# allenai/OLMoASR

Hardware: AMD Instinct MI355X
Metric: audio-seconds/sec/node (train step) (higher is better)
Workload: dtype bf16

## Files before the change

include/oasr_testing.h:

```cpp
#ifndef OASR_TESTING_H
#define OASR_TESTING_H
#include "oasr.h"
#ifdef __cplusplus
extern "C" {
#endif

int oasr_profile_gemm(int enable);
int oasr_gemm_set_variant(int v);
int oasr_decode_set_ln_fold(int mode);
int oasr_span_set_side_streams(int mode);
int oasr_span_side_streams(void);
int oasr_xcd_plan_debug(int d, int H, int Te, int M, int L, int team, int wg, int* out, int max_blocks);
int oasr_wide_supports_debug(int d, int H, int Te, int S_max, int L, int M, int nwg);
int oasr_wide_plan_debug(int d, int nwg, int N, int K, int wg, int wave, int* out, int max_units);
int oasr_xcd_offsets_ok_debug(const int64_t* layer0, long long lstride, long long cache_lstride, int d, int Te, int L, int M);
int oasr_attention_set_pingpong(int on);
int oasr_attention_set_span_grid(int on);
int oasr_gemm_set_stagger(int sleeps, int phases);
int oasr_gemm_force_general(int on);
int oasr_test_gemm(const oasr_gemm_args* a, float* colsum_scratch, int atomic_on_pp, int raster_gm, int stagger, int stagger_phases, void* stream);
int oasr_profile_gemm_records(char* buf, int cap);
int oasr_profile_gemm_collect(double* ms4, double* flops4, int64_t* count4, char* by_symbol , int cap);
int oasr_probe_lds_oob(const void* src_u16 , void* dst_u16 , void* stream);
int oasr_probe_tr16(const void* src_bf16 , void* dst_bf16 , void* stream);
int oasr_test_span_tables(const int32_t* span_host, int B, int S, const int64_t* targets, int32_t* rows_out, int32_t* span_out,
                          int64_t* targets_rows_out, int64_t* active_rows_out, void* stream);
int oasr_test_span_block_tables(const int32_t* span_host, int B, int S, int H, const int64_t* targets, int32_t* rows_out, int32_t* span_out,
                                int64_t* targets_rows_out, int32_t* blk128_out, int32_t* blk256_out, int32_t* counts_out, void* stream);

int oasr_test_embedding_fwd(const int64_t* tok, const float* E, const float* pos, void* x, int dtype, int B, int S, int d, int64_t n_embed,
                            const int32_t* rows, void* stream);
int oasr_test_embedding_bwd(const int64_t* tok, const void* dx, int dtype, float* dE, float* dpos, int B, int S, int d, int64_t pad_id,
                            int64_t n_embed, const int32_t* rows, const int32_t* span, void* stream);
int oasr_test_colsum(const void* x, int dtype, int64_t ld, int64_t M, int ncols, float* out, void* stream);
int oasr_test_conv2_col2im_dgelu(const void* dA, const void* u1, void* dpre1, int dtype, int B, int T1, int d, void* stream);
int oasr_test_conv1_col2im_mel(const void* dcol, int dtype, float* dmel, int B, int T1, int n_mels, void* stream);
int oasr_test_mel_to_time_major(const float* mel, void* out, int dtype, int B, int n_mels, int T, const float* clip_max, void* stream);
int oasr_test_pack_conv_weight(const float* w, void* dst, int dtype, int co, int ci, int ldk, void* stream);
int oasr_test_unpack_conv_grad(const float* g, float* dw, int co, int ci, int ldk, void* stream);
int oasr_test_pack_embedding(const float* e, void* dst, int rows, int rows_pad, int d, void* stream);
int oasr_test_dgelu_mul(const void* dy, const void* u, void* out, int dtype, int64_t n, void* stream);
int oasr_test_dlogits_from_f32(const float* src, int V, int64_t rows, int64_t ld, void* dst, int dtype, void* stream);
int oasr_test_logits_to_f32(const void* logits, int dtype, int64_t ld, int64_t rows, int V, float* out, void* stream);
int oasr_test_layernorm_bwd(const void* dy, const void* x, const float* gamma, const float* mean, const float* rstd, const void* dres, void* dx,
                            float* dgamma, float* dbeta, float* dsum, int dtype, int64_t rows, int d, void* stream);

int oasr_test_dtw_host(const float* cost, int64_t ld, int N, int M, int negate, int32_t* text_indices, int32_t* time_indices, int32_t* path_len,
                       void* workspace);

int oasr_test_argmax_rows(const void* logits, int dtype, int64_t ld, int V, int64_t n_rows, const int32_t* rows, const int32_t* span, int B, int S,
                          int32_t* pred_out, void* stream);

#ifdef __cplusplus
}
#endif
#endif
```

olmoasr_amd/_native.py:

```python
import ctypes as C
import os

import torch

_HERE = os.path.dirname(os.path.abspath(__file__))
LIB_PATH = os.environ.get("OASR_LIB") or os.path.join(_HERE, "liboasr.so")
_lib = None


class NativeError(RuntimeError):
    pass


class Dims(C.Structure):
    _fields_ = [(n, C.c_int) for n in ("n_mels", "n_audio_ctx", "n_audio_state", "n_audio_head", "n_audio_layer",
                                       "n_vocab", "n_text_ctx", "n_text_state", "n_text_head", "n_text_layer")]


class Operand(C.Structure):
    _fields_ = [("ptr", C.c_void_p), ("ld", C.c_int64), ("rpb", C.c_int), ("bstride", C.c_int64), ("lead", C.c_int),
                ("kvalid", C.c_int), ("trail_from", C.c_int)]


class GemmArgs(C.Structure):
# ... 25 lines not shown

class SpecAug(C.Structure):
    MAX_MASKS = 8
    _fields_ = [("freq_masks", C.c_int32), ("freq_width", C.c_int32), ("time_masks", C.c_int32), ("time_width", C.c_int32), ("fill", C.c_float)]


class EditArgs(C.Structure):
    MAX_LEN = 1023
    _fields_ = [("hyp", C.c_void_p), ("ref", C.c_void_p), ("hyp_len", C.c_void_p), ("ref_len", C.c_void_p), ("out", C.c_void_p),
                ("ld_hyp", C.c_int64), ("ld_ref", C.c_int64), ("B", C.c_int32), ("Lh", C.c_int32), ("Lr", C.c_int32), ("reserved", C.c_int32)]


class TrainStepArgs(C.Structure):
    _fields_ = [(n, C.c_void_p) for n in ("mel", "xa", "tokens", "targets", "text_len", "span_host", "mel_clip_max", "loss_out", "logits_out",
                                          "pred_out", "seg_events")] + \
               [(n, C.c_int32) for n in ("B", "S", "span_forward", "accumulate_loss")] + [("loss_scale", C.c_float), ("inv_accum", C.c_float)] + \
               [("label_smoothing", C.c_float), ("z_loss", C.c_float), ("loss_parts_out", C.c_void_p), ("loss_parts_rows", C.c_void_p)]


DTW_MAX_N, DTW_MAX_M = 448, 1500
ABI_VERSION = 216
KV_TAIL_BYTES = 327680
MODE_INFER, MODE_TRAIN, MODE_TRAIN_ENC, MODE_TRAIN_DEC = 0, 1, 2, 3
ROWTAB = 16
LORA_MAX_RANK = 64


def _declare(lib):
    vp, i32, i64, f32, sz = C.c_void_p, C.c_int, C.c_int64, C.c_float, C.c_size_t
    sig = {
        "oasr_last_error": (C.c_char_p, []),
        "oasr_version": (i32, []),
        "oasr_log_mel_workspace_bytes": (sz, [i32]),
        "oasr_log_mel": (i32, [vp, i32, i32, i32, vp, vp, vp]),
        "oasr_mel_filterbank": (i32, [vp]),
        "oasr_create": (vp, [C.POINTER(Dims)]),
        "oasr_create_ex": (vp, [C.POINTER(Dims), i32]),
        "oasr_create_ex2": (vp, [C.POINTER(Dims), i32, i32]),
        "oasr_compute_dtype": (i32, [vp]),
        "oasr_create_ex3": (vp, [C.POINTER(Dims), i32, i32, vp, i32, i32, f32]),
        "oasr_lora_count": (i32, [vp]),
        "oasr_lora_merge": (i32, [vp, vp]),
        "oasr_lora_merge_op": (i32, [vp, vp, vp, i32, i32, i32, f32, i32, vp, vp]),
        "oasr_lora_grad_scratch_bytes": (sz, [i32, i32, i32]),
        "oasr_lora_grad_op": (i32, [vp, vp, vp, i32, i32, i32, f32, vp, vp, vp, vp]),
        "oasr_encode": (i32, [vp, vp, i32, vp, vp, sz, vp]),
        "oasr_kv_cache_bytes": (sz, [vp, i32]),
        "oasr_decode_step_workspace_bytes": (sz, [vp, i32]),
        "oasr_decode_begin": (i32, [vp, vp, i32, vp, vp]),
        "oasr_decode_step": (i32, [vp, vp, i32, i32, vp, vp, vp, sz, vp]),
        "oasr_decode_check": (i32, [vp, i32, vp, vp]),
        "oasr_decode_logits": (i32, [vp, vp, vp, vp, i32, i32, i32, vp, vp, sz, vp]),
        "oasr_destroy": (None, [vp]),
        "oasr_param_count": (i32, [vp]),
        "oasr_param_info": (i32, [vp, i32, C.c_char_p, i32, C.POINTER(i64), C.POINTER(i64), C.POINTER(i32), C.POINTER(i64)]),
        "oasr_param_numel": (i64, [vp]),
        "oasr_segment_count": (i32, [vp]),
        "oasr_segment_info": (i32, [vp, i32, C.POINTER(i64), C.POINTER(i64)]),
        "oasr_bind": (i32, [vp, vp, vp, vp, vp, vp]),
        "oasr_shadow_bytes": (sz, [vp]),
        "oasr_bind_shadow": (i32, [vp, vp]),
        "oasr_refresh_shadow": (i32, [vp, vp]),
        "oasr_workspace_bytes": (sz, [vp, i32, i32, i32]),
        "oasr_forward": (i32, [vp, vp, vp, vp, i32, i32, vp, vp, vp, sz, vp]),
        "oasr_sizeof_train_step_args": (sz, []),
        "oasr_train_step": (i32, [vp, C.POINTER(TrainStepArgs), vp, sz, vp]),
        "oasr_log_mel_raw": (i32, [vp, i32, i32, i32, vp, vp, vp, vp]),
        "oasr_sizeof_attn_args": (sz, []),
        "oasr_test_span_tables": (i32, [vp, i32, i32, vp, vp, vp, vp, vp, vp]),
        "oasr_test_span_block_tables": (i32, [vp, i32, i32, i32, vp, vp, vp, vp, vp, vp, vp, vp]),
        "oasr_test_embedding_fwd": (i32, [vp, vp, vp, vp, i32, i32, i32, i32, i64, vp, vp]),
        "oasr_test_embedding_bwd": (i32, [vp, vp, i32, vp, vp, i32, i32, i32, i64, i64, vp, vp, vp]),
        "oasr_test_colsum": (i32, [vp, i32, i64, i64, i32, vp, vp]),
        "oasr_test_conv2_col2im_dgelu": (i32, [vp, vp, vp, i32, i32, i32, i32, vp]),
        "oasr_test_conv1_col2im_mel": (i32, [vp, i32, vp, i32, i32, i32, vp]),
        "oasr_test_mel_to_time_major": (i32, [vp, vp, i32, i32, i32, i32, vp, vp]),
        "oasr_test_pack_conv_weight": (i32, [vp, vp, i32, i32, i32, i32, vp]),
        "oasr_test_unpack_conv_grad": (i32, [vp, vp, i32, i32, i32, vp]),
        "oasr_test_pack_embedding": (i32, [vp, vp, i32, i32, i32, vp]),
        "oasr_test_dgelu_mul": (i32, [vp, vp, vp, i32, i64, vp]),
        "oasr_test_dlogits_from_f32": (i32, [vp, i32, i64, i64, vp, i32, vp]),
        "oasr_test_logits_to_f32": (i32, [vp, i32, i64, i64, i32, vp, vp]),
        "oasr_test_layernorm_bwd": (i32, [vp, vp, vp, vp, vp, vp, vp, vp, vp, vp, i32, i64, i32, vp]),
        "oasr_train_fwd": (i32, [vp, vp, vp, vp, i32, i32, vp, vp, sz, vp]),
        "oasr_train_bwd": (i32, [vp, vp, vp, vp, i32, i32, vp, vp, sz, vp]),
        "oasr_zero_grad": (i32, [vp, vp]),
        "oasr_train_encode": (i32, [vp, vp, i32, vp, vp, sz, vp]),
        "oasr_train_encode_bwd": (i32, [vp, vp, i32, vp, vp, sz, vp]),
        "oasr_train_decode": (i32, [vp, vp, vp, vp, i32, i32, vp, vp, sz, vp]),
        "oasr_train_decode_bwd": (i32, [vp, vp, vp, vp, i32, i32, vp, vp, sz, vp]),
        "oasr_set_trainable": (i32, [vp, vp, i32]),
        "oasr_optim_step": (i32, [vp, f32, f32, f32, f32, f32, f32, f32, i64, vp, vp, vp]),
        "oasr_grad_sumsq_range": (i32, [vp, i64, i64, vp, vp, vp]),
        "oasr_optim_step_range": (i32, [vp, i64, i64, vp, vp, vp, f32, f32, f32, f32, f32, f32, f32, i64, vp]),
        "oasr_gemm": (i32, [C.POINTER(GemmArgs), vp]),
        "oasr_test_gemm": (i32, [C.POINTER(GemmArgs), vp, i32, i32, i32, i32, vp]),
        "oasr_profile_gemm_records": (i32, [C.c_char_p, i32]),
        "oasr_layernorm_fwd": (i32, [vp, vp, vp, vp, vp, vp, i64, i32, vp]),
        "oasr_layernorm_bwd": (i32, [vp, vp, vp, vp, vp, vp, vp, vp, vp, i64, i32, vp]),
        "oasr_attention_fwd": (i32, [C.POINTER(AttnArgs), vp]),
        "oasr_attention_bwd": (i32, [C.POINTER(AttnArgs), vp]),
        "oasr_attention_scores": (i32, [C.POINTER(AttnArgs), i32, vp, vp]),
        "oasr_sizeof_align_args": (sz, []),
        "oasr_alignment_workspace_bytes": (sz, [i32, i32, i32]),
        "oasr_alignment_matrix": (i32, [C.POINTER(AlignArgs), vp, sz, vp]),
        "oasr_dtw_workspace_bytes": (sz, [i32, i32]),
        "oasr_dtw": (i32, [vp, i64, i32, i32, i32, vp, vp, vp, vp, sz, vp]),
        "oasr_test_dtw_host": (i32, [vp, i64, i32, i32, i32, vp, vp, vp, vp]),
        "oasr_sizeof_specaug": (sz, []),
        "oasr_spec_augment": (i32, [vp, i32, i32, i32, C.POINTER(SpecAug), C.c_uint64, C.c_uint64, vp]),
        "oasr_spec_augment_plan": (i32, [C.POINTER(SpecAug), C.c_uint64, C.c_uint64, i32, i32, vp, vp]),
        "oasr_sizeof_edit_args": (sz, []),
        "oasr_edit_counts": (i32, [C.POINTER(EditArgs), vp]),
        "oasr_edit_counts_host": (i32, [C.POINTER(EditArgs)]),
        "oasr_test_argmax_rows": (i32, [vp, i32, i64, i32, i64, vp, vp, i32, i32, vp, vp]),
        "oasr_cross_entropy": (i32, [vp, i64, i32, vp, i64, i64, f32, vp, vp, vp, i32, vp]),
        "oasr_cross_entropy_ex": (i32, [vp, i64, i32, vp, i64, i64, f32, vp, vp, vp, i32, f32, f32, vp, vp]),
        "oasr_cast_f32_bf16": (i32, [vp, vp, i64, vp]),
        "oasr_pick_tokens": (i32, [vp, i64, i32, i64, vp, vp, vp, vp, vp]),
        "oasr_pick_tokens_ts": (i32, [vp, i64, i32, i64, vp, vp, vp, i64, i32, i32, i32, i32, i32, vp, vp, vp]),
        "oasr_topk_tokens": (i32, [vp, i64, i32, i64, vp, vp, vp, i64, i32, i32, i32, i32, i32, i32, vp, vp, vp]),
        "oasr_sample_tokens": (i32, [vp, i64, i32, i64, vp, vp, vp, i64, i32, i32, i32, i32, i32, f32, vp, vp, vp, vp]),
        "oasr_probe_tr16": (i32, [vp, vp, vp]),
        "oasr_probe_lds_oob": (i32, [vp, vp, vp]),
        "oasr_profile_gemm": (i32, [i32]),
        "oasr_gemm_force_general": (i32, [i32]),
        "oasr_gemm_set_stagger": (i32, [i32, i32]),
        "oasr_gemm_set_variant": (i32, [i32]),
        "oasr_decode_set_ln_fold": (i32, [i32]),
        "oasr_span_set_side_streams": (i32, [i32]),
        "oasr_span_side_streams": (i32, []),
        "oasr_xcd_plan_debug": (i32, [i32, i32, i32, i32, i32, i32, i32, vp, i32]),
        "oasr_xcd_offsets_ok_debug": (i32, [vp, C.c_longlong, C.c_longlong, i32, i32, i32, i32]),
        "oasr_wide_supports_debug": (i32, [i32, i32, i32, i32, i32, i32, i32]),
        "oasr_wide_plan_debug": (i32, [i32, i32, i32, i32, i32, i32, vp, i32]),
        "oasr_attention_set_pingpong": (i32, [i32]),
        "oasr_attention_set_span_grid": (i32, [i32]),
        "oasr_profile_gemm_collect": (i32, [vp, vp, vp, C.c_char_p, i32]),
    }
    for name, (res, args) in sig.items():
        fn = getattr(lib, name)
        fn.restype = res
        fn.argtypes = args
    return list(sig)


EXPORTS = None


def lib():
    global _lib, EXPORTS
    if _lib is None:
        if not os.path.isfile(LIB_PATH):
            raise NativeError(f"{LIB_PATH} not found: run `python -c 'import __graft_entry__ as g; g.build()'` "
                              "(hipcc --offload-arch=gfx950).  There is no CPU/PyTorch fallback for this path.")
        try:
            _lib = C.CDLL(LIB_PATH)
        except OSError as e:
            raise NativeError(f"cannot load {LIB_PATH}: {e}") from e
        handle, _lib = _lib, None
        vfn = getattr(handle, "oasr_version", None)
        ver = int(vfn()) if vfn is not None else None
        sfn = getattr(handle, "oasr_sizeof_attn_args", None)
        size = int(sfn()) if sfn is not None else None
        if ver != ABI_VERSION or size != C.sizeof(AttnArgs):
            raise NativeError(f"{LIB_PATH}: ABI version {ver} / oasr_attn_args of {size} bytes, this binding is written for version "
# ... 48 lines not shown
```

olmoasr_amd/csrc/api.hip:

```cpp
#include <stdarg.h>

#include "../../include/oasr.h"
#include "kernels.h"

static thread_local char g_err[512] = "";

void oasr_set_error(const char* fmt, ...) {
  va_list ap;
  va_start(ap, fmt);
  vsnprintf(g_err, sizeof(g_err), fmt, ap);
  va_end(ap);
}

extern "C" const char* oasr_last_error(void) { return g_err; }
extern "C" int oasr_version(void) { return OASR_ABI_VERSION; }
extern "C" size_t oasr_sizeof_attn_args(void) { return sizeof(oasr_attn_args); }

static OperandView to_view(const oasr_operand& o) {
  return OperandView{(const bf16_t*)o.ptr, (long)o.ld, o.rpb, (long)o.bstride, o.lead, o.kvalid, o.trail_from};
}

static int to_gemm(const oasr_gemm_args* a, GemmArgs& g) {
  OASR_REQUIRE(a, "oasr_gemm: null args");
  g = gemm_defaults();
// ... 200 lines not shown
}

#define OASR_TEST_DTYPE(name) \
  OASR_REQUIRE(dtype == OASR_DTYPE_BF16 || dtype == OASR_DTYPE_F32, name ": dtype %d (0 = bf16, 1 = fp32 activations)", dtype)

extern "C" int oasr_test_embedding_fwd(const int64_t* tok, const float* E, const float* pos, void* x, int dtype, int B, int S, int d,
                                       int64_t n_embed, const int32_t* rows, void* stream) {
  OASR_TEST_DTYPE("oasr_test_embedding_fwd");
  if (dtype == OASR_DTYPE_BF16) return launch_embedding_fwd(tok, E, pos, (bf16_t*)x, B, S, d, (long)n_embed, (hipStream_t)stream, rows);
  return launch_embedding_fwd(tok, E, pos, (float*)x, B, S, d, (long)n_embed, (hipStream_t)stream, rows);
}
extern "C" int oasr_test_embedding_bwd(const int64_t* tok, const void* dx, int dtype, float* dE, float* dpos, int B, int S, int d, int64_t pad_id,
                                       int64_t n_embed, const int32_t* rows, const int32_t* span, void* stream) {
  OASR_TEST_DTYPE("oasr_test_embedding_bwd");
  OASR_REQUIRE(!span || rows, "oasr_test_embedding_bwd: span comes with a chunk-row table");
  if (dtype == OASR_DTYPE_BF16)
    return launch_embedding_bwd(tok, (const bf16_t*)dx, dE, dpos, B, S, d, (long)pad_id, (long)n_embed, (hipStream_t)stream, rows, span);
  return launch_embedding_bwd(tok, (const float*)dx, dE, dpos, B, S, d, (long)pad_id, (long)n_embed, (hipStream_t)stream, rows, span);
}
extern "C" int oasr_test_colsum(const void* x, int dtype, int64_t ld, int64_t M, int ncols, float* out, void* stream) {
  OASR_TEST_DTYPE("oasr_test_colsum");
  if (dtype == OASR_DTYPE_BF16) return launch_colsum_accum((const bf16_t*)x, (long)ld, (long)M, ncols, out, (hipStream_t)stream);
  return launch_colsum_accum((const float*)x, (long)ld, (long)M, ncols, out, (hipStream_t)stream);
}
extern "C" int oasr_test_conv2_col2im_dgelu(const void* dA, const void* u1, void* dpre1, int dtype, int B, int T1, int d, void* stream) {
  OASR_TEST_DTYPE("oasr_test_conv2_col2im_dgelu");
  OASR_REQUIRE(B > 0 && T1 > 0 && d > 0, "oasr_test_conv2_col2im_dgelu: bad shape (B=%d T1=%d d=%d)", B, T1, d);
  if (dtype == OASR_DTYPE_BF16) return launch_conv2_col2im_dgelu((const bf16_t*)dA, (const bf16_t*)u1, (bf16_t*)dpre1, B, T1, d, (hipStream_t)stream);
  return launch_conv2_col2im_dgelu((const float*)dA, (const float*)u1, (float*)dpre1, B, T1, d, (hipStream_t)stream);
}
extern "C" int oasr_test_conv1_col2im_mel(const void* dcol, int dtype, float* dmel, int B, int T1, int n_mels, void* stream) {
  OASR_TEST_DTYPE("oasr_test_conv1_col2im_mel");
  if (dtype == OASR_DTYPE_BF16) return launch_conv1_col2im_mel((const bf16_t*)dcol, dmel, B, T1, n_mels, (hipStream_t)stream);
  return launch_conv1_col2im_mel((const float*)dcol, dmel, B, T1, n_mels, (hipStream_t)stream);
}
extern "C" int oasr_test_mel_to_time_major(const float* mel, void* out, int dtype, int B, int n_mels, int T, const float* clip_max, void* stream) {
  OASR_TEST_DTYPE("oasr_test_mel_to_time_major");
  OASR_REQUIRE(B > 0 && n_mels > 0 && T > 0, "oasr_test_mel_to_time_major: bad shape (B=%d n_mels=%d T=%d)", B, n_mels, T);
  if (dtype == OASR_DTYPE_BF16) return launch_mel_to_time_major(mel, (bf16_t*)out, B, n_mels, T, (hipStream_t)stream, clip_max);
  return launch_mel_to_time_major(mel, (float*)out, B, n_mels, T, (hipStream_t)stream, clip_max);
}
extern "C" int oasr_test_pack_conv_weight(const float* w, void* dst, int dtype, int co, int ci, int ldk, void* stream) {
  OASR_TEST_DTYPE("oasr_test_pack_conv_weight");
  OASR_REQUIRE(co > 0 && ci > 0, "oasr_test_pack_conv_weight: bad shape (co=%d ci=%d)", co, ci);
  if (dtype == OASR_DTYPE_BF16) return launch_pack_conv_weight(w, (bf16_t*)dst, co, ci, ldk, (hipStream_t)stream);
  return launch_pack_conv_weight(w, (float*)dst, co, ci, ldk, (hipStream_t)stream);
}
extern "C" int oasr_test_unpack_conv_grad(const float* g, float* dw, int co, int ci, int ldk, void* stream) {
  OASR_REQUIRE(co > 0 && ci > 0, "oasr_test_unpack_conv_grad: bad shape (co=%d ci=%d)", co, ci);
  return launch_unpack_conv_grad(g, dw, co, ci, ldk, (hipStream_t)stream);
}
extern "C" int oasr_test_pack_embedding(const float* e, void* dst, int rows, int rows_pad, int d, void* stream) {
  OASR_REQUIRE(rows > 0 && d > 0, "oasr_test_pack_embedding: bad shape (rows=%d d=%d)", rows, d);
  return launch_pack_embedding(e, (bf16_t*)dst, rows, rows_pad, d, (hipStream_t)stream);
}
extern "C" int oasr_test_dgelu_mul(const void* dy, const void* u, void* out, int dtype, int64_t n, void* stream) {
  OASR_TEST_DTYPE("oasr_test_dgelu_mul");
  OASR_REQUIRE(n > 0, "oasr_test_dgelu_mul: n = %lld", (long long)n);
  if (dtype == OASR_DTYPE_BF16) return launch_dgelu_mul((const bf16_t*)dy, (const bf16_t*)u, (bf16_t*)out, (long)n, (hipStream_t)stream);
  return launch_dgelu_mul((const float*)dy, (const float*)u, (float*)out, (long)n, (hipStream_t)stream);
}
extern "C" int oasr_test_dlogits_from_f32(const float* src, int V, int64_t rows, int64_t ld, void* dst, int dtype, void* stream) {
  OASR_TEST_DTYPE("oasr_test_dlogits_from_f32");
  OASR_REQUIRE(rows > 0 && V > 0, "oasr_test_dlogits_from_f32: bad shape");
  if (dtype == OASR_DTYPE_BF16) return launch_dlogits_from_f32(src, V, (long)rows, (long)ld, (bf16_t*)dst, (hipStream_t)stream);
  return launch_dlogits_from_f32(src, V, (long)rows, (long)ld, (float*)dst, (hipStream_t)stream);
}
extern "C" int oasr_test_logits_to_f32(const void* logits, int dtype, int64_t ld, int64_t rows, int V, float* out, void* stream) {
  OASR_TEST_DTYPE("oasr_test_logits_to_f32");
  OASR_REQUIRE(logits && out && rows > 0 && V > 0 && V <= ld, "oasr_test_logits_to_f32: bad args");
  if (dtype == OASR_DTYPE_BF16) return launch_logits_to_f32((const bf16_t*)logits, (long)ld, (long)rows, V, out, (hipStream_t)stream);
  return launch_logits_to_f32((const float*)logits, (long)ld, (long)rows, V, out, (hipStream_t)stream);
}
extern "C" int oasr_test_layernorm_bwd(const void* dy, const void* x, const float* gamma, const float* mean, const float* rstd, const void* dres,
                                       void* dx, float* dgamma, float* dbeta, float* dsum, int dtype, int64_t rows, int d, void* stream) {
  OASR_TEST_DTYPE("oasr_test_layernorm_bwd");
  if (dtype == OASR_DTYPE_BF16)
    return launch_layernorm_bwd((const bf16_t*)dy, (const bf16_t*)x, gamma, mean, rstd, (const bf16_t*)dres, (bf16_t*)dx, dgamma, dbeta, dsum,
                                (long)rows, d, (hipStream_t)stream);
  return launch_layernorm_bwd((const float*)dy, (const float*)x, gamma, mean, rstd, (const float*)dres, (float*)dx, dgamma, dbeta, dsum, (long)rows, d,
                              (hipStream_t)stream);
}

extern "C" int oasr_test_argmax_rows(const void* logits, int dtype, int64_t ld, int V, int64_t n_rows, const int32_t* rows, const int32_t* span, int B,
                                     int S, int32_t* pred_out, void* stream) {
  OASR_TEST_DTYPE("oasr_test_argmax_rows");
  if (dtype == OASR_DTYPE_BF16)
    return launch_argmax_rows((const bf16_t*)logits, (long)ld, V, (long)n_rows, rows, span, B, S, pred_out, (hipStream_t)stream);
  return launch_argmax_rows((const float*)logits, (long)ld, V, (long)n_rows, rows, span, B, S, pred_out, (hipStream_t)stream);
}

extern "C" int oasr_cross_entropy_ex(void* logits, int64_t ld, int V, const int64_t* targets, int64_t rows, int64_t ignore, float gscale,
                                     int32_t* n_valid_dev, float* row_loss, float* loss_out, int write_grad, float label_smoothing, float z_loss,
                                     float* row_parts, void* stream) {
  hipStream_t st = (hipStream_t)stream;
  int rc = check_ce_reg("oasr_cross_entropy_ex", label_smoothing, z_loss);
  if (rc) return rc;
  CeReg reg;
  reg.eps = label_smoothing;
  reg.z = z_loss;
  reg.parts = row_parts;
  reg.parts_stride = (long)rows;
  rc = launch_count_valid(targets, rows, ignore, V, n_valid_dev, st);
  if (rc) return rc;
  rc = launch_cross_entropy((bf16_t*)logits, ld, V, targets, rows, ignore, gscale, n_valid_dev, row_loss, write_grad, st, reg);
  if (rc) return rc;
  if (loss_out) rc = launch_loss_reduce(row_loss, rows, n_valid_dev, 1.0f, loss_out, 0, st);
  return rc;
}
extern "C" int oasr_cross_entropy(void* logits, int64_t ld, int V, const int64_t* targets, int64_t rows, int64_t ignore, float gscale,
                                  int32_t* n_valid_dev, float* row_loss, float* loss_out, int write_grad, void* stream) {
  return oasr_cross_entropy_ex(logits, ld, V, targets, rows, ignore, gscale, n_valid_dev, row_loss, loss_out, write_grad, 0.f, 0.f, nullptr, stream);
}

extern "C" int oasr_pick_tokens(const float* logits, int64_t ld, int V, int64_t rows, const float* mask, const float* mask2, int64_t* tok,
                                float* logprob, void* stream) {
  return launch_pick_tokens(logits, ld, V, rows, mask, mask2, tok, logprob, (hipStream_t)stream);
}

extern "C" int oasr_pick_tokens_ts(const float* logits, int64_t ld, int V, int64_t rows, const float* mask, const float* mask2,
                                   const int64_t* history, int64_t history_ld, int n_history, int timestamp_begin, int eot, int no_timestamps,
                                   int max_initial_index, int64_t* tok, float* logprob, void* stream) {
  return launch_pick_tokens_ts(logits, ld, V, rows, mask, mask2, history, history_ld, n_history, timestamp_begin, eot, no_timestamps,
                               max_initial_index, tok, logprob, (hipStream_t)stream);
}

extern "C" int oasr_topk_tokens(const float* logits, int64_t ld, int V, int64_t rows, const float* mask, const float* mask2,
                                const int64_t* history, int64_t history_ld, int n_history, int timestamp_begin, int eot, int no_timestamps,
                                int max_initial_index, int K, int64_t* tok, float* logprob, void* stream) {
  return launch_topk_tokens_ts(logits, ld, V, rows, mask, mask2, history, history_ld, n_history, timestamp_begin, eot, no_timestamps,
                               max_initial_index, K, tok, logprob, (hipStream_t)stream);
}
extern "C" int oasr_sample_tokens(const float* logits, int64_t ld, int V, int64_t rows, const float* mask, const float* mask2,
                                  const int64_t* history, int64_t history_ld, int n_history, int timestamp_begin, int eot, int no_timestamps,
                                  int max_initial_index, float temperature, const float* uniforms, int64_t* tok, float* logprob, void* stream) {
  return launch_sample_tokens_ts(logits, ld, V, rows, mask, mask2, history, history_ld, n_history, timestamp_begin, eot, no_timestamps,
                                 max_initial_index, temperature, uniforms, tok, logprob, (hipStream_t)stream);
}

extern "C" int oasr_cast_f32_bf16(const float* src, void* dst, int64_t n, void* stream) {
  return launch_cast_f32_bf16(src, (bf16_t*)dst, n, (hipStream_t)stream);
}

typedef __attribute__((address_space(3))) s16x4_t* lds_s16x4_ptr_t;
__global__ void probe_tr16_kernel(const bf16_t* __restrict__ src, bf16_t* __restrict__ dst) {
  __shared__ __attribute__((aligned(16))) bf16_t tile[16 * 64];
  const int l = threadIdx.x;
  for (int i = l; i < 16 * 64; i += 64) tile[i] = src[i];
  __syncthreads();
  const int row = (l >> 4) * 4 + ((l & 15) >> 2), col = ((l & 15) & 3) * 4;
  const s16x4_t v = __builtin_amdgcn_ds_read_tr16_b64_v4i16((lds_s16x4_ptr_t)(tile + row * 64 + col));
  for (int j = 0; j < 4; ++j) dst[l * 4 + j] = (bf16_t)v[j];
}
typedef __attribute__((address_space(3))) void* lds_void_ptr_t;
__global__ void probe_lds_oob_kernel(const bf16_t* __restrict__ src, bf16_t* __restrict__ dst) {
  __shared__ __attribute__((aligned(16))) bf16_t tile[64 * 8];
  const int l = threadIdx.x;
  for (int i = l; i < 64 * 8; i += 64) tile[i] = 0xAAAA;
  __syncthreads();
  const __amdgpu_buffer_rsrc_t rs = __builtin_amdgcn_make_buffer_rsrc(const_cast<bf16_t*>(src), 0, 64 * 16, 0x00020000);
  const unsigned off = l < 32 ? l * 16 : 0x80000000u;
  __builtin_amdgcn_raw_ptr_buffer_load_lds(rs, (lds_void_ptr_t)tile, 16, off, 0, 0, 0);
  __syncthreads();
  for (int i = l; i < 64 * 8; i += 64) dst[i] = tile[i];
}
extern "C" int oasr_probe_lds_oob(const void* src, void* dst, void* stream) {
// ... 10 lines not shown
```

olmoasr_amd/csrc/norm.hip:

```cpp
#include "kernels.h"

namespace {

constexpr int MAXC = 4;

__device__ __forceinline__ void unpack8(const u32x4_t& p, float (&f)[8]) {
#pragma unroll
  for (int i = 0; i < 4; ++i) {
    f[2 * i] = bf_lo(p[i]);
    f[2 * i + 1] = bf_hi(p[i]);
  }
}
__device__ __forceinline__ u32x4_t pack8(const float (&f)[8]) {
  u32x4_t p;
#pragma unroll
  for (int i = 0; i < 4; ++i) p[i] = pack_bf2(f[2 * i], f[2 * i + 1]);
  return p;
}

__global__ __launch_bounds__(256) void ln_fwd_kernel(const bf16_t* __restrict__ x, const float* __restrict__ gamma,
                                                     const float* __restrict__ beta, bf16_t* __restrict__ y,
                                                     float* __restrict__ mean_out, float* __restrict__ rstd_out, long rows,
                                                     int d) {
  const int lane = threadIdx.x & 63;
  const long row = (long)blockIdx.x * 4 + (threadIdx.x >> 6);
  if (row >= rows) return;
  const int nchunk = d >> 3;
  float v[MAXC][8];
  float s = 0.f;
#pragma unroll
  for (int c = 0; c < MAXC; ++c) {
    const int ch = lane + 64 * c;
    if (ch < nchunk) {
      unpack8(*(const u32x4_t*)(x + row * d + ch * 8), v[c]);
#pragma unroll
      for (int i = 0; i < 8; ++i) s += v[c][i];
    }
  }
  const float mean = wave_sum(s) / (float)d;
  float q = 0.f;
#pragma unroll
  for (int c = 0; c < MAXC; ++c) {
    const int ch = lane + 64 * c;
    if (ch < nchunk) {
#pragma unroll
      for (int i = 0; i < 8; ++i) {
        const float t = v[c][i] - mean;
        q += t * t;
      }
    }
  }
  const float var = wave_sum(q) / (float)d;
  const float rstd = rsqrtf(var + 1e-5f);
#pragma unroll
  for (int c = 0; c < MAXC; ++c) {
    const int ch = lane + 64 * c;
    if (ch < nchunk) {
      float o[8];
      const f32x4_t g0 = *(const f32x4_t*)(gamma + ch * 8), g1 = *(const f32x4_t*)(gamma + ch * 8 + 4);
      const f32x4_t b0 = *(const f32x4_t*)(beta + ch * 8), b1 = *(const f32x4_t*)(beta + ch * 8 + 4);
#pragma unroll
      for (int i = 0; i < 4; ++i) {
        o[i] = (v[c][i] - mean) * rstd * g0[i] + b0[i];
        o[4 + i] = (v[c][4 + i] - mean) * rstd * g1[i] + b1[i];
      }
      *(u32x4_t*)(y + row * d + ch * 8) = pack8(o);
    }
  }
  if (lane == 0) {
    if (mean_out) mean_out[row] = mean;
    if (rstd_out) rstd_out[row] = rstd;
  }
}

template <int NCH, int PG>
__global__ __launch_bounds__(256) void ln_bwd_kernel(const bf16_t* __restrict__ dy, const bf16_t* __restrict__ x,
                                                     const float* __restrict__ gamma, const float* __restrict__ mean,
                                                     const float* __restrict__ rstd, const bf16_t* __restrict__ dres,
                                                     bf16_t* __restrict__ dx, float* __restrict__ dgamma,
                                                     float* __restrict__ dbeta, float* __restrict__ dsum, long rows, int d) {
  __shared__ float red[4][512 * NCH];
  const int lane = threadIdx.x & 63, wave = threadIdx.x >> 6;
  const int nchunk = d >> 3;
  float gw[NCH][8], dg[NCH][8], db[NCH][8], dsx[NCH][8];
#pragma unroll
  for (int c = 0; c < NCH; ++c) {
    const int ch = lane + 64 * c;
#pragma unroll
    for (int i = 0; i < 8; ++i) {
      dg[c][i] = 0.f;
      db[c][i] = 0.f;
      dsx[c][i] = 0.f;
      gw[c][i] = (ch < nchunk) ? gamma[ch * 8 + i] : 0.f;
    }
  }
  const float inv_d = 1.0f / (float)d;
  const long stride = (long)gridDim.x * 4;
  for (long row0 = (long)blockIdx.x * 4 + wave; row0 < rows; row0 += 2 * stride) {
    u32x4_t px[2][NCH], pd[2][NCH], pr[2][NCH];
    bool live[2];
#pragma unroll
    for (int r = 0; r < 2; ++r) {
      const long row = row0 + r * stride;
      live[r] = row < rows;
      const long rr = live[r] ? row : row0;
#pragma unroll
      for (int c = 0; c < NCH; ++c) {
        const int ch = lane + 64 * c;
        if (ch < nchunk) {
          px[r][c] = *(const u32x4_t*)(x + rr * d + ch * 8);
          pd[r][c] = *(const u32x4_t*)(dy + rr * d + ch * 8);
          if (dres) pr[r][c] = *(const u32x4_t*)(dres + rr * d + ch * 8);
        }
      }
    }
#pragma unroll
    for (int r = 0; r < 2; ++r) {
      if (!live[r]) continue;
      const long row = row0 + r * stride;
      const float mu = mean[row], rs = rstd[row];
      float xh[NCH][8], gy[NCH][8];
      float s1 = 0.f, s2 = 0.f;
#pragma unroll
      for (int c = 0; c < NCH; ++c) {
        const int ch = lane + 64 * c;
        if (ch < nchunk) {
          float xv[8], dv[8];
          unpack8(px[r][c], xv);
          unpack8(pd[r][c], dv);
#pragma unroll
          for (int i = 0; i < 8; ++i) {
            xh[c][i] = (xv[i] - mu) * rs;
            gy[c][i] = dv[i] * gw[c][i];
            s1 += gy[c][i];
            s2 += gy[c][i] * xh[c][i];
            if (PG & 1) dg[c][i] += dv[i] * xh[c][i];
            if (PG & 2) db[c][i] += dv[i];
          }
        }
      }
      s1 = wave_sum(s1) * inv_d;
      s2 = wave_sum(s2) * inv_d;
#pragma unroll
      for (int c = 0; c < NCH; ++c) {
        const int ch = lane + 64 * c;
        if (ch < nchunk) {
          float o[8];
#pragma unroll
          for (int i = 0; i < 8; ++i) o[i] = rs * (gy[c][i] - s1 - xh[c][i] * s2);
          if (dres) {
            float rv[8];
            unpack8(pr[r][c], rv);
#pragma unroll
            for (int i = 0; i < 8; ++i) o[i] = bf_round(o[i]) + rv[i];
          }
          const u32x4_t packed = pack8(o);
          *(u32x4_t*)(dx + row * d + ch * 8) = packed;
          if (dsum) {
#pragma unroll
            for (int i = 0; i < 4; ++i) {
              dsx[c][2 * i] += bf_lo(packed[i]);
              dsx[c][2 * i + 1] += bf_hi(packed[i]);
            }
          }
        }
      }
    }
  }
  for (int pass = 0; pass < (dsum ? 3 : 2); ++pass) {
    if ((pass == 0 && !(PG & 1)) || (pass == 1 && !(PG & 2))) continue;
#pragma unroll
    for (int c = 0; c < NCH; ++c) {
      const int ch = lane + 64 * c;
      if (ch < nchunk) {
#pragma unroll
        for (int i = 0; i < 8; ++i) red[wave][ch * 8 + i] = pass == 0 ? dg[c][i] : (pass == 1 ? db[c][i] : dsx[c][i]);
      }
    }
    __syncthreads();
    float* dst = pass == 0 ? dgamma : (pass == 1 ? dbeta : dsum);
    for (int j = threadIdx.x; j < d; j += 256) {
      const float t = red[0][j] + red[1][j] + red[2][j] + red[3][j];
      unsafeAtomicAdd(dst + j, t);
    }
    __syncthreads();
  }
}

}

int launch_layernorm_fwd(const bf16_t* x, const float* gamma, const float* beta, bf16_t* y, float* mean, float* rstd,
                         long rows, int d, hipStream_t s) {
  OASR_REQUIRE(x && gamma && beta && y, "layernorm_fwd: null pointer");
  OASR_REQUIRE(d % 8 == 0 && d <= 2048 && d > 0, "layernorm: d=%d must be a multiple of 8 and <= 2048", d);
  if (rows <= 0) return OASR_OK;
  hipLaunchKernelGGL(ln_fwd_kernel, dim3((unsigned)((rows + 3) / 4)), dim3(256), 0, s, x, gamma, beta, y, mean, rstd, rows, d);
  OASR_LAUNCH_CHECK();
  return OASR_OK;
}

template <int PG>
static void ln_bwd_launch(dim3 grid, const bf16_t* dy, const bf16_t* x, const float* gamma, const float* mean, const float* rstd,
                          const bf16_t* dres, bf16_t* dx, float* dgamma, float* dbeta, float* dsum, long rows, int d, hipStream_t s) {
  if (d <= 512)
    hipLaunchKernelGGL((ln_bwd_kernel<1, PG>), grid, dim3(256), 0, s, dy, x, gamma, mean, rstd, dres, dx, dgamma, dbeta, dsum, rows, d);
  else if (d <= 1024)
    hipLaunchKernelGGL((ln_bwd_kernel<2, PG>), grid, dim3(256), 0, s, dy, x, gamma, mean, rstd, dres, dx, dgamma, dbeta, dsum, rows, d);
  else if (d <= 1536)
    hipLaunchKernelGGL((ln_bwd_kernel<3, PG>), grid, dim3(256), 0, s, dy, x, gamma, mean, rstd, dres, dx, dgamma, dbeta, dsum, rows, d);
  else
    hipLaunchKernelGGL((ln_bwd_kernel<4, PG>), grid, dim3(256), 0, s, dy, x, gamma, mean, rstd, dres, dx, dgamma, dbeta, dsum, rows, d);
}

int launch_layernorm_bwd(const bf16_t* dy, const bf16_t* x, const float* gamma, const float* mean, const float* rstd,
                         const bf16_t* dres, bf16_t* dx, float* dgamma, float* dbeta, float* dsum, long rows, int d, hipStream_t s) {
  OASR_REQUIRE(dy && x && gamma && mean && rstd && dx, "layernorm_bwd: null pointer");
  OASR_REQUIRE(d % 8 == 0 && d <= 2048 && d > 0, "layernorm: d=%d must be a multiple of 8 and <= 2048", d);
  if (rows <= 0) return OASR_OK;
  long blocks = (rows + 3) / 4;
  if (blocks > 512) blocks = 512;
  const dim3 grid((unsigned)blocks);
  switch ((dgamma ? 1 : 0) | (dbeta ? 2 : 0)) {
    case 3: ln_bwd_launch<3>(grid, dy, x, gamma, mean, rstd, dres, dx, dgamma, dbeta, dsum, rows, d, s); break;
    case 2: ln_bwd_launch<2>(grid, dy, x, gamma, mean, rstd, dres, dx, dgamma, dbeta, dsum, rows, d, s); break;
    case 1: ln_bwd_launch<1>(grid, dy, x, gamma, mean, rstd, dres, dx, dgamma, dbeta, dsum, rows, d, s); break;
    default: ln_bwd_launch<0>(grid, dy, x, gamma, mean, rstd, dres, dx, dgamma, dbeta, dsum, rows, d, s); break;
  }
  OASR_LAUNCH_CHECK();
  return OASR_OK;
}
```

Before: 6270.

## Software-pipeline layernorm forward and backward with persistent grids and nontemporal access

The layernorm forward kernel becomes a persistent grid-stride kernel capped at a fixed number of workgroups. It hoists gamma and beta into registers and prefetches the next row while the current one is normalized. The backward kernel gets the same multi-stage prefetch pipeline, templated rows-per-group and a residual flag. It also uses nontemporal loads and stores and lowers the grid cap from 512 to 256 workgroups. The aim is to hide global-memory latency in these bandwidth-bound kernels, at the cost of more register pressure and possibly lower occupancy and parallelism.

```diff
diff --git a/include/oasr_testing.h b/include/oasr_testing.h
--- a/include/oasr_testing.h
+++ b/include/oasr_testing.h
@@ -44,6 +44,7 @@
 int oasr_test_logits_to_f32(const void* logits, int dtype, int64_t ld, int64_t rows, int V, float* out, void* stream);
 int oasr_test_layernorm_bwd(const void* dy, const void* x, const float* gamma, const float* mean, const float* rstd, const void* dres, void* dx,
                             float* dgamma, float* dbeta, float* dsum, int dtype, int64_t rows, int d, void* stream);
+int oasr_test_layernorm_walk(int d, int64_t* out3);
 
 int oasr_test_dtw_host(const float* cost, int64_t ld, int N, int M, int negate, int32_t* text_indices, int32_t* time_indices, int32_t* path_len,
                        void* workspace);
diff --git a/olmoasr_amd/_native.py b/olmoasr_amd/_native.py
--- a/olmoasr_amd/_native.py
+++ b/olmoasr_amd/_native.py
@@ -131,6 +131,7 @@
         "oasr_test_dlogits_from_f32": (i32, [vp, i32, i64, i64, vp, i32, vp]),
         "oasr_test_logits_to_f32": (i32, [vp, i32, i64, i64, i32, vp, vp]),
         "oasr_test_layernorm_bwd": (i32, [vp, vp, vp, vp, vp, vp, vp, vp, vp, vp, i32, i64, i32, vp]),
+        "oasr_test_layernorm_walk": (i32, [i32, C.POINTER(i64)]),
         "oasr_train_fwd": (i32, [vp, vp, vp, vp, i32, i32, vp, vp, sz, vp]),
         "oasr_train_bwd": (i32, [vp, vp, vp, vp, i32, i32, vp, vp, sz, vp]),
         "oasr_zero_grad": (i32, [vp, vp]),
diff --git a/olmoasr_amd/csrc/api.hip b/olmoasr_amd/csrc/api.hip
--- a/olmoasr_amd/csrc/api.hip
+++ b/olmoasr_amd/csrc/api.hip
@@ -306,6 +306,19 @@
                               (hipStream_t)stream);
 }
 
+void layernorm_walk(int d, long* fwd_sweep, long* bwd_sweep, int* bwd_group);
+extern "C" int oasr_test_layernorm_walk(int d, int64_t* out3) {
+  OASR_HOOK_GATE("oasr_test_layernorm_walk");
+  OASR_REQUIRE(out3 && d > 0 && d <= 2048 && d % 8 == 0, "oasr_test_layernorm_walk: bad args (d=%d)", d);
+  long f = 0, b = 0;
+  int g = 0;
+  layernorm_walk(d, &f, &b, &g);
+  out3[0] = f;
+  out3[1] = b;
+  out3[2] = g;
+  return OASR_OK;
+}
+
 extern "C" int oasr_test_argmax_rows(const void* logits, int dtype, int64_t ld, int V, int64_t n_rows, const int32_t* rows, const int32_t* span, int B,
                                      int S, int32_t* pred_out, void* stream) {
   OASR_TEST_DTYPE("oasr_test_argmax_rows");
diff --git a/olmoasr_amd/csrc/norm.hip b/olmoasr_amd/csrc/norm.hip
--- a/olmoasr_amd/csrc/norm.hip
+++ b/olmoasr_amd/csrc/norm.hip
@@ -1,8 +1,6 @@
 #include "kernels.h"
 
 namespace {
-
-constexpr int MAXC = 4;
 
 __device__ __forceinline__ void unpack8(const u32x4_t& p, float (&f)[8]) {
 #pragma unroll
@@ -18,21 +16,67 @@
   return p;
 }
 
-__global__ __launch_bounds__(256) void ln_fwd_kernel(const bf16_t* __restrict__ x, const float* __restrict__ gamma,
-                                                     const float* __restrict__ beta, bf16_t* __restrict__ y,
-                                                     float* __restrict__ mean_out, float* __restrict__ rstd_out, long rows,
-                                                     int d) {
-  const int lane = threadIdx.x & 63;
-  const long row = (long)blockIdx.x * 4 + (threadIdx.x >> 6);
-  if (row >= rows) return;
-  const int nchunk = d >> 3;
-  float v[MAXC][8];
+#ifndef OASR_LN_FWD_WGS
+#define OASR_LN_FWD_WGS 1024
+#endif
+#ifndef OASR_LN_BWD_WGS
+#define OASR_LN_BWD_WGS 256
+#endif
+#ifndef OASR_LN_FWD_DEPTH
+#define OASR_LN_FWD_DEPTH 2
+#endif
+#ifndef OASR_LN_BWD_RPG
+#define OASR_LN_BWD_RPG 2
+#endif
+#ifndef OASR_LN_BWD_DEPTH
+#define OASR_LN_BWD_DEPTH 2
+#endif
+#ifndef OASR_LN_NT
+#define OASR_LN_NT 29
+#endif
+constexpr int LN_CUS = 256;
+constexpr int LN_FWD_WGS = OASR_LN_FWD_WGS;
+constexpr int LN_BWD_WGS = OASR_LN_BWD_WGS;
+constexpr int ln_nch(int d) { return d <= 512 ? 1 : d <= 1024 ? 2 : d <= 1536 ? 3 : 4; }
+constexpr int ln_bwd_rpg(int nch) { return nch <= 2 ? OASR_LN_BWD_RPG : 1; }
+constexpr int ln_bwd_depth(int nch) { return nch <= 2 ? OASR_LN_BWD_DEPTH : 2; }
+
+template <bool NT>
+__device__ __forceinline__ u32x4_t ld16(const bf16_t* p) {
+  return NT ? __builtin_nontemporal_load((const u32x4_t*)p) : *(const u32x4_t*)p;
+}
+template <bool NT>
+__device__ __forceinline__ void st16(bf16_t* p, const u32x4_t& v) {
+  if (NT)
+    __builtin_nontemporal_store(v, (u32x4_t*)p);
+  else
+    *(u32x4_t*)p = v;
+}
+
+template <int NCH>
+__device__ __forceinline__ void ln_fwd_load(u32x4_t (&p)[NCH], const bf16_t* __restrict__ x, long row, int d, int lane, int nchunk) {
+#pragma unroll
+  for (int c = 0; c < NCH; ++c) {
+    const int ch = lane + 64 * c;
+    p[c] = ld16<(OASR_LN_NT >> 3) & 1>((x + row * d) + (unsigned)((ch < nchunk ? ch : nchunk - 1) * 8));
+  }
+}
+__device__ __forceinline__ void ln_landed(const u32x4_t& v) { asm volatile("" ::"v"(v)); }
+__device__ __forceinline__ void ln_landed(float v) { asm volatile("" ::"v"(v)); }
+
+template <int NCH>
+__device__ __forceinline__ void ln_fwd_row(const u32x4_t (&p)[NCH], const f32x4_t (&g0)[NCH], const f32x4_t (&g1)[NCH],
+                                           const f32x4_t (&b0)[NCH], const f32x4_t (&b1)[NCH], bf16_t* __restrict__ y,
+                                           float* __restrict__ mean_out, float* __restrict__ rstd_out, long row, int d, int lane, int nchunk) {
+#pragma unroll
+  for (int c = 0; c < NCH; ++c) ln_landed(p[c]);
+  float v[NCH][8];
   float s = 0.f;
 #pragma unroll
-  for (int c = 0; c < MAXC; ++c) {
+  for (int c = 0; c < NCH; ++c) {
     const int ch = lane + 64 * c;
     if (ch < nchunk) {
-      unpack8(*(const u32x4_t*)(x + row * d + ch * 8), v[c]);
+      unpack8(p[c], v[c]);
 #pragma unroll
       for (int i = 0; i < 8; ++i) s += v[c][i];
     }
@@ -40,7 +84,7 @@
   const float mean = wave_sum(s) / (float)d;
   float q = 0.f;
 #pragma unroll
-  for (int c = 0; c < MAXC; ++c) {
+  for (int c = 0; c < NCH; ++c) {
     const int ch = lane + 64 * c;
     if (ch < nchunk) {
 #pragma unroll
@@ -53,18 +97,16 @@
   const float var = wave_sum(q) / (float)d;
   const float rstd = rsqrtf(var + 1e-5f);
 #pragma unroll
-  for (int c = 0; c < MAXC; ++c) {
+  for (int c = 0; c < NCH; ++c) {
     const int ch = lane + 64 * c;
     if (ch < nchunk) {
       float o[8];
-      const f32x4_t g0 = *(const f32x4_t*)(gamma + ch * 8), g1 = *(const f32x4_t*)(gamma + ch * 8 + 4);
-      const f32x4_t b0 = *(const f32x4_t*)(beta + ch * 8), b1 = *(const f32x4_t*)(beta + ch * 8 + 4);
 #pragma unroll
       for (int i = 0; i < 4; ++i) {
-        o[i] = (v[c][i] - mean) * rstd * g0[i] + b0[i];
-        o[4 + i] = (v[c][4 + i] - mean) * rstd * g1[i] + b1[i];
-      }
-      *(u32x4_t*)(y + row * d + ch * 8) = pack8(o);
+        o[i] = (v[c][i] - mean) * rstd * g0[c][i] + b0[c][i];
+        o[4 + i] = (v[c][4 + i] - mean) * rstd * g1[c][i] + b1[c][i];
+      }
+      st16<(OASR_LN_NT >> 4) & 1>((y + row * d) + (unsigned)(ch * 8), pack8(o));
     }
   }
   if (lane == 0) {
@@ -73,15 +115,86 @@
   }
 }
 
-template <int NCH, int PG>
-__global__ __launch_bounds__(256) void ln_bwd_kernel(const bf16_t* __restrict__ dy, const bf16_t* __restrict__ x,
+template <int NCH, int DEPTH>
+__global__ __launch_bounds__(256) void ln_fwd_kernel(const bf16_t* __restrict__ x, const float* __restrict__ gamma,
+                                                     const float* __restrict__ beta, bf16_t* __restrict__ y,
+                                                     float* __restrict__ mean_out, float* __restrict__ rstd_out, long rows, int d) {
+  const int lane = threadIdx.x & 63;
+  const int nchunk = d >> 3;
+  const long stride = (long)gridDim.x * 4;
+  long row = (long)blockIdx.x * 4 + __builtin_amdgcn_readfirstlane(threadIdx.x >> 6);
+  if (row >= rows) return;
+  f32x4_t g0[NCH], g1[NCH], b0[NCH], b1[NCH];
+#pragma unroll
+  for (int c = 0; c < NCH; ++c) {
+    const int ch = lane + 64 * c;
+    const int at = (ch < nchunk ? ch : nchunk - 1) * 8;
+    g0[c] = *(const f32x4_t*)(gamma + at);
+    g1[c] = *(const f32x4_t*)(gamma + at + 4);
+    b0[c] = *(const f32x4_t*)(beta + at);
+    b1[c] = *(const f32x4_t*)(beta + at + 4);
+  }
+  __builtin_amdgcn_sched_barrier(0);
+  u32x4_t p[DEPTH][NCH];
+#pragma unroll
+  for (int k = 0; k < DEPTH - 1; ++k) ln_fwd_load<NCH>(p[k], x, row + k * stride < rows ? row + k * stride : row, d, lane, nchunk);
+  while (row + (DEPTH - 1) * stride < rows) {
+#pragma unroll
+    for (int k = 0; k < DEPTH; ++k) {
+      const long ahead = row + (DEPTH - 1) * stride;
+      ln_fwd_load<NCH>(p[(k + DEPTH - 1) % DEPTH], x, ahead < rows ? ahead : row, d, lane, nchunk);
+      __builtin_amdgcn_sched_barrier(0);
+      ln_fwd_row<NCH>(p[k], g0, g1, b0, b1, y, mean_out, rstd_out, row, d, lane, nchunk);
+      row += stride;
+    }
+  }
+#pragma unroll
+  for (int k = 0; k < DEPTH - 1; ++k) {
+    if (row < rows) ln_fwd_row<NCH>(p[k], g0, g1, b0, b1, y, mean_out, rstd_out, row, d, lane, nchunk);
+    row += stride;
+  }
+}
+
+template <int NCH, int RPG, bool RES>
+struct LnBwdStage {
+  u32x4_t px[RPG][NCH], pd[RPG][NCH], pr[RPG][RES ? NCH : 1];
+  float mu[RPG], rs[RPG];
+};
+
+template <int NCH, int RPG, bool RES>
+__device__ __forceinline__ void ln_bwd_load(LnBwdStage<NCH, RPG, RES>& st, const bf16_t* __restrict__ dy, const bf16_t* __restrict__ x,
+                                            const float* __restrict__ mean, const float* __restrict__ rstd,
+                                            const bf16_t* __restrict__ dres, long row0, long stride, long rows, int d, int lane, int nchunk, int vzero) {
+#pragma unroll
+  for (int r = 0; r < RPG; ++r) {
+    const long row = row0 + r * stride;
+    const long rr = row < rows ? row : row0;
+#pragma unroll
+    for (int c = 0; c < NCH; ++c) {
+      const int ch = lane + 64 * c;
+      const unsigned at = (unsigned)((ch < nchunk ? ch : nchunk - 1) * 8);
+      st.px[r][c] = ld16<(OASR_LN_NT >> 1) & 1>((x + rr * d) + at);
+      st.pd[r][c] = ld16<OASR_LN_NT & 1>((dy + rr * d) + at);
+      if (RES) st.pr[r][c] = ld16<OASR_LN_NT & 1>((dres + rr * d) + at);
+    }
+    st.mu[r] = mean[rr + vzero];
+    st.rs[r] = rstd[rr + vzero];
+  }
+}
+
+template <int NCH, int PG, int RPG, int DEPTH, bool RES>
+__global__ __launch_bounds__(256, (NCH <= 2 && LN_BWD_WGS > LN_CUS) ? 2 : 1) void ln_bwd_kernel(const bf16_t* __restrict__ dy, const bf16_t* __restrict__ x,
                                                      const float* __restrict__ gamma, const float* __restrict__ mean,
                                                      const float* __restrict__ rstd, const bf16_t* __restrict__ dres,
                                                      bf16_t* __restrict__ dx, float* __restrict__ dgamma,
                                                      float* __restrict__ dbeta, float* __restrict__ dsum, long rows, int d) {
   __shared__ float red[4][512 * NCH];
-  const int lane = threadIdx.x & 63, wave = threadIdx.x >> 6;
+  const int lane = threadIdx.x & 63, wave = __builtin_amdgcn_readfirstlane(threadIdx.x >> 6);
+  const int vzero = (int)(threadIdx.x >> 6) - wave;
   const int nchunk = d >> 3;
+  const long stride = (long)gridDim.x * 4;
+  const long step = RPG * stride;
+  long row0 = (long)blockIdx.x * 4 + wave;
   float gw[NCH][8], dg[NCH][8], db[NCH][8], dsx[NCH][8];
 #pragma unroll
   for (int c = 0; c < NCH; ++c) {
@@ -94,31 +207,28 @@
       gw[c][i] = (ch < nchunk) ? gamma[ch * 8 + i] : 0.f;
     }
   }
+  __builtin_amdgcn_sched_barrier(0);
+  LnBwdStage<NCH, RPG, RES> st[DEPTH];
+  if (row0 < rows) {
+#pragma unroll
+    for (int k = 0; k < DEPTH - 1; ++k)
+      ln_bwd_load<NCH, RPG, RES>(st[k], dy, x, mean, rstd, dres, row0 + k * step < rows ? row0 + k * step : row0, stride, rows, d, lane, nchunk, vzero);
+  }
   const float inv_d = 1.0f / (float)d;
-  const long stride = (long)gridDim.x * 4;
-  for (long row0 = (long)blockIdx.x * 4 + wave; row0 < rows; row0 += 2 * stride) {
-    u32x4_t px[2][NCH], pd[2][NCH], pr[2][NCH];
-    bool live[2];
-#pragma unroll
-    for (int r = 0; r < 2; ++r) {
-      const long row = row0 + r * stride;
-      live[r] = row < rows;
-      const long rr = live[r] ? row : row0;
+  auto reduce_store = [&](const LnBwdStage<NCH, RPG, RES>& sg, long g0) {
+#pragma unroll
+    for (int r = 0; r < RPG; ++r) {
+      const long row = g0 + r * stride;
+      if (RPG > 1 && row >= rows) continue;
 #pragma unroll
       for (int c = 0; c < NCH; ++c) {
-        const int ch = lane + 64 * c;
-        if (ch < nchunk) {
-          px[r][c] = *(const u32x4_t*)(x + rr * d + ch * 8);
-          pd[r][c] = *(const u32x4_t*)(dy + rr * d + ch * 8);
-          if (dres) pr[r][c] = *(const u32x4_t*)(dres + rr * d + ch * 8);
-        }
-      }
-    }
-#pragma unroll
-    for (int r = 0; r < 2; ++r) {
-      if (!live[r]) continue;
-      const long row = row0 + r * stride;
-      const float mu = mean[row], rs = rstd[row];
+        ln_landed(sg.px[r][c]);
+        ln_landed(sg.pd[r][c]);
+        if (RES) ln_landed(sg.pr[r][c]);
+      }
+      ln_landed(sg.mu[r]);
+      ln_landed(sg.rs[r]);
+      const float mu = sg.mu[r], rs = sg.rs[r];
       float xh[NCH][8], gy[NCH][8];
       float s1 = 0.f, s2 = 0.f;
 #pragma unroll
@@ -126,8 +236,8 @@
         const int ch = lane + 64 * c;
         if (ch < nchunk) {
           float xv[8], dv[8];
-          unpack8(px[r][c], xv);
-          unpack8(pd[r][c], dv);
+          unpack8(sg.px[r][c], xv);
+          unpack8(sg.pd[r][c], dv);
 #pragma unroll
           for (int i = 0; i < 8; ++i) {
             xh[c][i] = (xv[i] - mu) * rs;
@@ -150,12 +260,12 @@
           for (int i = 0; i < 8; ++i) o[i] = rs * (gy[c][i] - s1 - xh[c][i] * s2);
           if (dres) {
             float rv[8];
-            unpack8(pr[r][c], rv);
+            unpack8(sg.pr[r][RES ? c : 0], rv);
 #pragma unroll
             for (int i = 0; i < 8; ++i) o[i] = bf_round(o[i]) + rv[i];
           }
           const u32x4_t packed = pack8(o);
-          *(u32x4_t*)(dx + row * d + ch * 8) = packed;
+          st16<(OASR_LN_NT >> 2) & 1>((dx + row * d) + (unsigned)(ch * 8), packed);
           if (dsum) {
 #pragma unroll
             for (int i = 0; i < 4; ++i) {
@@ -166,6 +276,21 @@
         }
       }
     }
+  };
+  while (row0 + (DEPTH - 1) * step < rows) {
+#pragma unroll
+    for (int k = 0; k < DEPTH; ++k) {
+      const long ahead = row0 + (DEPTH - 1) * step;
+      ln_bwd_load<NCH, RPG, RES>(st[(k + DEPTH - 1) % DEPTH], dy, x, mean, rstd, dres, ahead < rows ? ahead : row0, stride, rows, d, lane, nchunk, vzero);
+      __builtin_amdgcn_sched_barrier(0);
+      reduce_store(st[k], row0);
+      row0 += step;
+    }
+  }
+#pragma unroll
+  for (int k = 0; k < DEPTH - 1; ++k) {
+    if (row0 < rows) reduce_store(st[k], row0);
+    row0 += step;
   }
   for (int pass = 0; pass < (dsum ? 3 : 2); ++pass) {
     if ((pass == 0 && !(PG & 1)) || (pass == 1 && !(PG & 2))) continue;
@@ -194,22 +319,38 @@
   OASR_REQUIRE(x && gamma && beta && y, "layernorm_fwd: null pointer");
   OASR_REQUIRE(d % 8 == 0 && d <= 2048 && d > 0, "layernorm: d=%d must be a multiple of 8 and <= 2048", d);
   if (rows <= 0) return OASR_OK;
-  hipLaunchKernelGGL(ln_fwd_kernel, dim3((unsigned)((rows + 3) / 4)), dim3(256), 0, s, x, gamma, beta, y, mean, rstd, rows, d);
+  long blocks = (rows + 3) / 4;
+  if (blocks > LN_FWD_WGS) blocks = LN_FWD_WGS;
+  const dim3 grid((unsigned)blocks);
+  switch (ln_nch(d)) {
+    case 1: hipLaunchKernelGGL((ln_fwd_kernel<1, OASR_LN_FWD_DEPTH>), grid, dim3(256), 0, s, x, gamma, beta, y, mean, rstd, rows, d); break;
+    case 2: hipLaunchKernelGGL((ln_fwd_kernel<2, OASR_LN_FWD_DEPTH>), grid, dim3(256), 0, s, x, gamma, beta, y, mean, rstd, rows, d); break;
+    case 3: hipLaunchKernelGGL((ln_fwd_kernel<3, OASR_LN_FWD_DEPTH>), grid, dim3(256), 0, s, x, gamma, beta, y, mean, rstd, rows, d); break;
+    default: hipLaunchKernelGGL((ln_fwd_kernel<4, OASR_LN_FWD_DEPTH>), grid, dim3(256), 0, s, x, gamma, beta, y, mean, rstd, rows, d); break;
+  }
   OASR_LAUNCH_CHECK();
   return OASR_OK;
+}
+
+template <int NCH, int PG>
+static void ln_bwd_launch_nch(dim3 grid, const bf16_t* dy, const bf16_t* x, const float* gamma, const float* mean, const float* rstd,
+                              const bf16_t* dres, bf16_t* dx, float* dgamma, float* dbeta, float* dsum, long rows, int d, hipStream_t s) {
+  constexpr int RPG = ln_bwd_rpg(NCH), DEPTH = ln_bwd_depth(NCH);
+  if (dres)
+    hipLaunchKernelGGL((ln_bwd_kernel<NCH, PG, RPG, DEPTH, true>), grid, dim3(256), 0, s, dy, x, gamma, mean, rstd, dres, dx, dgamma, dbeta, dsum, rows, d);
+  else
+    hipLaunchKernelGGL((ln_bwd_kernel<NCH, PG, RPG, DEPTH, false>), grid, dim3(256), 0, s, dy, x, gamma, mean, rstd, dres, dx, dgamma, dbeta, dsum, rows, d);
 }
 
 template <int PG>
 static void ln_bwd_launch(dim3 grid, const bf16_t* dy, const bf16_t* x, const float* gamma, const float* mean, const float* rstd,
                           const bf16_t* dres, bf16_t* dx, float* dgamma, float* dbeta, float* dsum, long rows, int d, hipStream_t s) {
-  if (d <= 512)
-    hipLaunchKernelGGL((ln_bwd_kernel<1, PG>), grid, dim3(256), 0, s, dy, x, gamma, mean, rstd, dres, dx, dgamma, dbeta, dsum, rows, d);
-  else if (d <= 1024)
-    hipLaunchKernelGGL((ln_bwd_kernel<2, PG>), grid, dim3(256), 0, s, dy, x, gamma, mean, rstd, dres, dx, dgamma, dbeta, dsum, rows, d);
-  else if (d <= 1536)
-    hipLaunchKernelGGL((ln_bwd_kernel<3, PG>), grid, dim3(256), 0, s, dy, x, gamma, mean, rstd, dres, dx, dgamma, dbeta, dsum, rows, d);
-  else
-    hipLaunchKernelGGL((ln_bwd_kernel<4, PG>), grid, dim3(256), 0, s, dy, x, gamma, mean, rstd, dres, dx, dgamma, dbeta, dsum, rows, d);
+  switch (ln_nch(d)) {
+    case 1: ln_bwd_launch_nch<1, PG>(grid, dy, x, gamma, mean, rstd, dres, dx, dgamma, dbeta, dsum, rows, d, s); break;
+    case 2: ln_bwd_launch_nch<2, PG>(grid, dy, x, gamma, mean, rstd, dres, dx, dgamma, dbeta, dsum, rows, d, s); break;
+    case 3: ln_bwd_launch_nch<3, PG>(grid, dy, x, gamma, mean, rstd, dres, dx, dgamma, dbeta, dsum, rows, d, s); break;
+    default: ln_bwd_launch_nch<4, PG>(grid, dy, x, gamma, mean, rstd, dres, dx, dgamma, dbeta, dsum, rows, d, s); break;
+  }
 }
 
 int launch_layernorm_bwd(const bf16_t* dy, const bf16_t* x, const float* gamma, const float* mean, const float* rstd,
@@ -218,7 +359,7 @@
   OASR_REQUIRE(d % 8 == 0 && d <= 2048 && d > 0, "layernorm: d=%d must be a multiple of 8 and <= 2048", d);
   if (rows <= 0) return OASR_OK;
   long blocks = (rows + 3) / 4;
-  if (blocks > 512) blocks = 512;
+  if (blocks > LN_BWD_WGS) blocks = LN_BWD_WGS;
   const dim3 grid((unsigned)blocks);
   switch ((dgamma ? 1 : 0) | (dbeta ? 2 : 0)) {
     case 3: ln_bwd_launch<3>(grid, dy, x, gamma, mean, rstd, dres, dx, dgamma, dbeta, dsum, rows, d, s); break;
@@ -229,3 +370,9 @@
   OASR_LAUNCH_CHECK();
   return OASR_OK;
 }
+
+void layernorm_walk(int d, long* fwd_sweep, long* bwd_sweep, int* bwd_group) {
+  *bwd_group = ln_bwd_rpg(ln_nch(d));
+  *fwd_sweep = (long)LN_FWD_WGS * 4;
+  *bwd_sweep = (long)LN_BWD_WGS * 4 * *bwd_group;
+}
```

New measurement: 6280, median of 6. About the same (+0.2%).
